# retab-dev/k-LLMs

Hardware: AMD Instinct MI355X
Metric: end_to_end_consensus_requests_per_s (higher is better)
Workload: dtype bf16; 1 GPU; model=llama-3-8b, n=5, mode=create, global_batch=24, seq_len=512, parallelism=dp1 tp1

## Files before the change

### kllms_amd/engine/engine.py

```python

from __future__ import annotations

import os
import time
from dataclasses import dataclass, field
from typing import Any, List, Optional, Tuple

import torch

from ..models.llama import ForwardBatch
from .config import EngineConfig, ModelArchConfig
from .kvcache import PagedKVCache, SequenceKV
from .sampling import SamplingParams
from .shared_prefix import build_shared_prefix_tiles
from .tokenizer import BaseTokenizer, load_tokenizer
from .. import ops


@dataclass
class GenRequest:
    prompt_ids: List[int]
    n: int = 1
    sampling: SamplingParams = field(default_factory=SamplingParams)
    constraint: Optional[Any] = None
# ... 492 lines not shown
            kv_caches=self.kv.layer_caches(),
            **attn,
        )
        hidden = self.model.forward_hidden(torch.tensor(all_ids, dtype=torch.long, device=dev), batch)
        return self.model.compute_logits(hidden[torch.tensor(last_rows, device=dev)])

    def _alloc_with_prefix(self, ids: List[int], prefix_blocks: List[int]) -> SequenceKV:
        if not prefix_blocks:
            return self.kv.alloc_sequence(len(ids))
        bs = self.kv.block_size
        n_total = (len(ids) + bs - 1) // bs
        seq = SequenceKV(blocks=[], num_tokens=len(ids))
        try:
            for b in prefix_blocks:
                self.kv.allocator.incref(b)
                seq.blocks.append(b)
            for _ in range(n_total - len(prefix_blocks)):
                seq.blocks.append(self.kv.allocator.alloc())
        except Exception:
            for b in seq.blocks:
                self.kv.allocator.free(b)
            seq.blocks = []
            raise
        return seq

    def _fork_and_sample(
        self,
        requests: List[GenRequest],
        parent_seqs: List[SequenceKV],
        prefill_logits: torch.Tensor,
        streams: List[_Stream],
    ) -> List[_Stream]:
        new_streams: List[_Stream] = []
        for ri, req in enumerate(requests):
            rid = self._seed_counter
            self._seed_counter += 1
            base_seed = req.sampling.seed if req.sampling.seed is not None else (self.config.seed * 1000003 + rid)
            fork_id = self._fork_counter
            self._fork_counter += 1
            for si in range(max(1, req.n)):
                seq = self.kv.fork(parent_seqs[ri])
                cstate = req.constraint.init_state() if req.constraint is not None else None
                st = _Stream(ri, si, seq, req.sampling, seed=base_seed + 7919 * si,
                             constraint=req.constraint, constraint_state=cstate,
                             fork_id=fork_id)
                st.deadline = req.deadline if self.ctx.world_size == 1 else None
                streams.append(st)
                new_streams.append(st)
            self.kv.free_sequence(parent_seqs[ri])

        rep_logits = torch.cat([
            prefill_logits[ri].unsqueeze(0).expand(max(1, requests[ri].n), -1)
            for ri in range(len(requests))
        ])
        self._sample_and_append(rep_logits.contiguous(), new_streams)
        return new_streams

    def prefill_chunk(
        self, seq: SequenceKV, prompt_ids: List[int], start: int, end: int, want_logits: bool = False
    ) -> Optional[torch.Tensor]:
        dev = self.device
        ids = torch.tensor(prompt_ids[start:end], dtype=torch.long, device=dev)
        pos = torch.arange(start, end, dtype=torch.long, device=dev)
        slots_all = self.kv.prefill_slot_mapping(seq)
        slots = torch.tensor(slots_all[start:end], dtype=torch.long, device=dev)
        if self.paged_prefill_attention:
            attn = dict(extend=ops.build_paged_prefill(
                [end - start], [start], [seq.blocks], dev, self.kv.block_size))
        else:
            nb = len(seq.blocks)
            bt = (
                torch.tensor(seq.blocks, dtype=torch.int32, device=dev)
                .unsqueeze(0).expand(end - start, nb).contiguous()
            )
            attn = dict(block_tables=bt,
                        context_lens=torch.arange(start + 1, end + 1, dtype=torch.int32, device=dev))
        batch = ForwardBatch(
            mode="decode",
            positions=pos,
            slot_mapping=slots,
            kv_caches=self.kv.layer_caches(),
            **attn,
# ... 296 lines not shown
```

### kllms_amd/engine/kvcache.py

```python

from __future__ import annotations

import hashlib
from array import array
from collections import OrderedDict
from dataclasses import dataclass, field
from typing import Callable, List, Optional, Tuple

import torch


class BlockAllocator:
    def __init__(self, num_blocks: int):
        self.num_blocks = num_blocks
        self._free: list[int] = list(range(num_blocks - 1, -1, -1))
        self._refcount = [0] * num_blocks
        self.on_pressure: Optional[Callable[[], None]] = None

    @property
    def num_free(self) -> int:
        return len(self._free)

    def alloc(self) -> int:
        if not self._free and self.on_pressure is not None:
            self.on_pressure()
        if not self._free:
            raise RuntimeError("KV cache out of blocks")
        b = self._free.pop()
        assert self._refcount[b] == 0
        self._refcount[b] = 1
        return b

    def incref(self, block: int) -> None:
        assert self._refcount[block] > 0
        self._refcount[block] += 1

    def free(self, block: int) -> None:
        assert self._refcount[block] > 0
        self._refcount[block] -= 1
        if self._refcount[block] == 0:
            self._free.append(block)

# ... 26 lines not shown
        self.k_all = torch.zeros(num_layers, num_blocks, num_kv_heads, block_size, head_dim,
                                 device=device, dtype=dtype)
        self.v_all = torch.zeros_like(self.k_all)
        self.k_caches = [self.k_all[i] for i in range(num_layers)]
        self.v_caches = [self.v_all[i] for i in range(num_layers)]
        self.fp8 = dtype == torch.float8_e4m3fn
        if self.fp8:
            self.k_scale_all = torch.ones(num_layers, num_blocks, num_kv_heads, block_size,
                                          device=device, dtype=torch.float32)
            self.v_scale_all = torch.ones_like(self.k_scale_all)
        else:
            self.k_scale_all = self.v_scale_all = None
        self.allocator = BlockAllocator(num_blocks)

    def layer_caches(self) -> List[Tuple[torch.Tensor, torch.Tensor, Optional[torch.Tensor], Optional[torch.Tensor]]]:
        if self.fp8:
            return [(self.k_caches[i], self.v_caches[i], self.k_scale_all[i], self.v_scale_all[i])
                    for i in range(self.num_layers)]
        return [(self.k_caches[i], self.v_caches[i], None, None) for i in range(self.num_layers)]

    def alloc_sequence(self, num_tokens: int) -> SequenceKV:
        n_blocks = (num_tokens + self.block_size - 1) // self.block_size
        blocks: List[int] = []
        try:
            for _ in range(n_blocks):
                blocks.append(self.allocator.alloc())
        except Exception:
            for b in blocks:
                self.allocator.free(b)
            raise
        return SequenceKV(blocks=blocks, num_tokens=num_tokens)

    def fork(self, parent: SequenceKV) -> SequenceKV:
        child = SequenceKV(blocks=[], num_tokens=parent.num_tokens)
        tail = parent.num_tokens % self.block_size
        try:
            for i, b in enumerate(parent.blocks):
                if i == len(parent.blocks) - 1 and tail != 0:
                    child.blocks.append(self._copy_block(b))
                else:
                    self.allocator.incref(b)
                    child.blocks.append(b)
        except Exception:
            for b in child.blocks:
                self.allocator.free(b)
            child.blocks = []
            raise
        return child

    def _copy_block(self, src: int) -> int:
        dst = self.allocator.alloc()
        self.k_all[:, dst].copy_(self.k_all[:, src])
        self.v_all[:, dst].copy_(self.v_all[:, src])
        if self.fp8:
            self.k_scale_all[:, dst].copy_(self.k_scale_all[:, src])
            self.v_scale_all[:, dst].copy_(self.v_scale_all[:, src])
        return dst

    def append_slot(self, seq: SequenceKV) -> int:
        pos = seq.num_tokens
        off = pos % self.block_size
        blk_idx = pos // self.block_size
        if blk_idx == len(seq.blocks):
            seq.blocks.append(self.allocator.alloc())
        else:
            last = seq.blocks[blk_idx]
            if self.allocator.refcount(last) > 1:
                new = self._copy_block(last)
                self.allocator.free(last)
                seq.blocks[blk_idx] = new
        seq.num_tokens += 1
        return seq.blocks[blk_idx] * self.block_size + off

    def prefill_slot_mapping(self, seq: SequenceKV, start: int = 0) -> list[int]:
        slots = []
        for pos in range(start, seq.num_tokens):
            slots.append(seq.blocks[pos // self.block_size] * self.block_size + pos % self.block_size)
        return slots

    def free_sequence(self, seq: SequenceKV) -> None:
        for b in seq.blocks:
            self.allocator.free(b)
        seq.blocks = []
        seq.num_tokens = 0


class PrefixCache:

    def __init__(self, kv: "PagedKVCache", max_blocks: int):
# ... 64 lines not shown
```

### kllms_amd/models/llama.py

```python

from __future__ import annotations

import math
from dataclasses import dataclass
from typing import List, Literal, Optional, Tuple

import torch
import torch.nn as nn

from .. import ops
from ..engine.config import ModelArchConfig
from ..ops.torch_ref import build_cos_sin_cache
from ..parallel.tp import ColumnParallelLinear, ParallelContext, RowParallelLinear


@dataclass
class ForwardBatch:
    mode: Literal["prefill", "decode"]
    positions: torch.Tensor
    slot_mapping: torch.Tensor
    kv_caches: List[Tuple]
    cu_seqlens: Optional[torch.Tensor] = None
    block_tables: Optional[torch.Tensor] = None
    context_lens: Optional[torch.Tensor] = None
    shared: Optional["ops.SharedPrefix"] = None
    extend: Optional["ops.PagedPrefill"] = None


class LlamaAttention(nn.Module):
    def __init__(self, cfg: ModelArchConfig, ctx: ParallelContext, layer_idx: int, dtype):
        super().__init__()
        self.layer_idx = layer_idx
        tp = ctx.world_size
        assert cfg.num_heads % tp == 0 and cfg.num_kv_heads % tp == 0
        self.num_heads = cfg.num_heads // tp
        self.num_kv_heads = cfg.num_kv_heads // tp
        self.head_dim = cfg.head_dim_
        self.scale = 1.0 / math.sqrt(self.head_dim)
        q_size = cfg.num_heads * self.head_dim
        kv_size = cfg.num_kv_heads * self.head_dim
        self.qkv_proj = ColumnParallelLinear(
            cfg.hidden_size, q_size + 2 * kv_size, ctx, dtype=dtype,
            partition_sizes=[q_size, kv_size, kv_size],
            bias=cfg.attention_qkv_bias,
        )
        self.o_proj = RowParallelLinear(q_size, cfg.hidden_size, ctx, dtype=dtype)
        self._q = self.num_heads * self.head_dim
        self._kv = self.num_kv_heads * self.head_dim

    def forward(self, hidden: torch.Tensor, batch: ForwardBatch, cos_sin: torch.Tensor) -> torch.Tensor:
        T = hidden.shape[0]
        qkv = self.qkv_proj(hidden)
        q, k, v = qkv.split([self._q, self._kv, self._kv], dim=-1)
        q = q.view(T, self.num_heads, self.head_dim)
        k = k.view(T, self.num_kv_heads, self.head_dim)
        v = v.view(T, self.num_kv_heads, self.head_dim)
        ops.rope_inplace(q, k, batch.positions, cos_sin)

        k_cache, v_cache, k_scale, v_scale = batch.kv_caches[self.layer_idx]
        ops.store_kv(k, v, k_cache, v_cache, batch.slot_mapping, k_scale, v_scale)

        if batch.mode == "prefill":
            out = ops.attn_prefill_varlen(q, k, v, batch.cu_seqlens, self.scale)
        elif batch.extend is not None:
            out = ops.attn_prefill_paged(
                q, k_cache, v_cache, batch.extend, self.scale, k_scale, v_scale)
        else:
            out = ops.attn_decode_paged(
                q, k_cache, v_cache, batch.block_tables, batch.context_lens, self.scale,
                k_scale, v_scale, shared=batch.shared,
            )
        return self.o_proj(out.reshape(T, -1))


class LlamaMLP(nn.Module):
    def __init__(self, cfg: ModelArchConfig, ctx: ParallelContext, dtype):
        super().__init__()
        self.gate_up_proj = ColumnParallelLinear(
            cfg.hidden_size, 2 * cfg.intermediate_size, ctx, dtype=dtype,
            partition_sizes=[cfg.intermediate_size, cfg.intermediate_size],
        )
        self.down_proj = RowParallelLinear(cfg.intermediate_size, cfg.hidden_size, ctx, dtype=dtype)
        self._i = cfg.intermediate_size // ctx.world_size

    def forward(self, x: torch.Tensor) -> torch.Tensor:
        gate_up = self.gate_up_proj(x)
        gate, up = gate_up.split([self._i, self._i], dim=-1)
        return self.down_proj(ops.silu_mul(gate, up))


class RMSNormModule(nn.Module):
    def __init__(self, hidden_size: int, eps: float, dtype):
        super().__init__()
# ... 141 lines not shown
```

### kllms_amd/ops/__init__.py

```python

from __future__ import annotations

import os
from dataclasses import dataclass
from typing import Optional, Tuple

import torch

from . import torch_ref

_C = None
_C_err: Optional[str] = None
try:
    from kllms_amd import _C
except Exception as e:
    _C = None
    _C_err = str(e)


def hip_available() -> bool:
    return _C is not None


def _force_torch() -> bool:
# ... 94 lines not shown
        if x.dtype != torch.bfloat16:
            raise ValueError(f"linear_fp8w_batched on GPU needs bf16 activations, got {x.dtype}")
        if _fp8w_batched_kernel_takes(x, E, N, K):
            out = torch.empty((E, x.shape[-2], N), dtype=torch.bfloat16, device=x.device)
            C.linear_fp8w_batched(out, x, q, scale)
            return out
        if K % 16 == 0:
            w = torch.empty((E, N, K), dtype=torch.bfloat16, device=x.device)
            C.dequant_fp8w(w, q.view(E * N, K), scale.view(E * N))
        else:
            w = (q.float() * scale.unsqueeze(-1)).bfloat16()
        xb = x.unsqueeze(0).expand(E, -1, -1) if x.dim() == 2 else x
        return torch.bmm(xb, w.transpose(1, 2))
    return torch_ref.linear_fp8w_batched(x, q, scale)


def store_kv(
    k: torch.Tensor,
    v: torch.Tensor,
    k_cache: torch.Tensor,
    v_cache: torch.Tensor,
    slot_mapping: torch.Tensor,
    k_scale: Optional[torch.Tensor] = None,
    v_scale: Optional[torch.Tensor] = None,
) -> None:
    if k.is_cuda and not _force_torch():
        none = torch.empty(0, dtype=torch.float32, device=k.device)
        _hip_or_raise().store_kv(
            k, v, k_cache, v_cache, slot_mapping,
            k_scale if k_scale is not None else none,
            v_scale if v_scale is not None else none)
        return
    torch_ref.store_kv(k, v, k_cache, v_cache, slot_mapping, k_scale, v_scale)


def _prefill_tiles(cu_seqlens: torch.Tensor, device) -> tuple:
    NW = 8
    cu = cu_seqlens.cpu().tolist()
    grp_start, grp_len, grp_qpos0 = [], [], []
    for i in range(len(cu) - 1):
        s, e = cu[i], cu[i + 1]
        L = e - s
        tiles = list(range(0, L, 32))
        for g0 in range(0, len(tiles), NW):
            grp_start.append(s)
            grp_len.append(L)
            grp = tiles[g0 : g0 + NW]
            grp_qpos0.extend(grp + [-1] * (NW - len(grp)))
    t = lambda x: torch.tensor(x, dtype=torch.int32, device=device)
    return t(grp_start), t(grp_qpos0), t(grp_len)


def attn_prefill_varlen(
    q: torch.Tensor, k: torch.Tensor, v: torch.Tensor, cu_seqlens: torch.Tensor, scale: float
) -> torch.Tensor:
    if q.is_cuda and not _force_torch():
        out = torch.empty(q.shape, dtype=q.dtype, device=q.device)
        gs, gq, gl = _prefill_tiles(cu_seqlens, q.device)
        _hip_or_raise().attn_prefill(out, q, k, v, gs, gq, gl, scale)
        return out
    return torch_ref.attn_prefill_varlen(q, k, v, cu_seqlens, scale)


@dataclass
class SharedPrefix:

# ... 217 lines not shown
```

### kllms_amd/ops/hip/bindings.hip

```cpp

#include <torch/extension.h>
#include <ATen/hip/HIPContext.h>

#include "common.h"

extern "C" __global__ void rmsnorm_kernel(bf16_t*, const bf16_t*, const bf16_t*, int, float);
extern "C" __global__ void fused_add_rmsnorm_kernel(bf16_t*, const bf16_t*, bf16_t*, const bf16_t*, int, float);
extern "C" __global__ void silu_mul_kernel(bf16_t*, const bf16_t*, const bf16_t*, int64_t, int, int);
extern "C" __global__ void rope_kernel(bf16_t*, bf16_t*, const int64_t*, const float*, int, int, int, int, int);
extern "C" __global__ void store_kv_kernel(const bf16_t*, const bf16_t*, bf16_t*, bf16_t*, const int64_t*, int, int, int, int, int);
extern "C" __global__ void store_kv_fp8_kernel(const bf16_t*, const bf16_t*, unsigned char*, unsigned char*, float*, float*, const int64_t*, int, int, int, int, int);
extern "C" void launch_attn_decode_partial(float*, const bf16_t*, const void*, const void*, const float*, const float*, const int*, const int*, const int*, float, int, int, int, int, int, int, int, int, int, hipStream_t);
extern "C" void launch_attn_decode_shared(float*, const bf16_t*, const void*, const void*, const float*, const float*, const int*, const int*, const int*, const int*, float, int, int, int, int, int, int, int, int, int, int, hipStream_t);
extern "C" void launch_attn_prefill_paged(bf16_t*, const bf16_t*, const void*, const void*, const float*, const float*, const int*, const int*, const int*, const int*, const int*, float, int, int, int, int, int, int, int, int, int, int, hipStream_t);
extern "C" __global__ void attn_decode_reduce_kernel(bf16_t*, const float*, const int*, int, int, int, int);
extern "C" __global__ void attn_prefill_kernel(bf16_t*, const bf16_t*, const bf16_t*, const bf16_t*, const int*, const int*, const int*, float, int, int, int, int);
extern "C" __global__ void sample_kernel(int64_t*, float*, const float*, const float*, const float*, const int*, const int64_t*, const int64_t*, const uint32_t*, int, float*);
extern "C" __global__ void sample_fsm_kernel(int64_t*, float*, const float*, const float*, const float*, const int*, const int64_t*, const int64_t*, int32_t*, const int64_t*, int, int);
extern "C" __global__ void mfma_selftest_kernel(float*, const bf16_t*, const bf16_t*);

#define CHECK_BF16_CONTIG(t) \
  TORCH_CHECK((t).is_cuda() && (t).is_contiguous() && (t).scalar_type() == at::kBFloat16, #t " must be contiguous bf16 on GPU")

#define CHECK_KV_CACHE(t) \
  TORCH_CHECK((t).is_cuda() && (t).is_contiguous() && \
              ((t).scalar_type() == at::kBFloat16 || (t).scalar_type() == at::kFloat8_e4m3fn), \
              #t " must be a contiguous bf16 or fp8-e4m3 KV cache on GPU")

#define CHECK_BF16_ROWS(t) \
  TORCH_CHECK((t).is_cuda() && (t).scalar_type() == at::kBFloat16 && (t).dim() == 3 && \
              (t).stride(2) == 1 && (t).stride(1) == (t).size(2), #t " must be a bf16 [T,H,D] row view")

static inline hipStream_t cur_stream() {
  return at::hip::getCurrentHIPStream().stream();
}

static bf16_t* bf(torch::Tensor& t) { return reinterpret_cast<bf16_t*>(t.data_ptr()); }
static const bf16_t* cbf(const torch::Tensor& t) { return reinterpret_cast<const bf16_t*>(t.data_ptr()); }

void rmsnorm(torch::Tensor out, torch::Tensor in, torch::Tensor weight, double eps) {
  CHECK_BF16_CONTIG(out); CHECK_BF16_CONTIG(in); CHECK_BF16_CONTIG(weight);
  const int n = in.size(-1);
  TORCH_CHECK(n % 8 == 0, "hidden size must be a multiple of 8");
  const int rows = in.numel() / n;
// ... 28 lines not shown
  CHECK_BF16_ROWS(q); CHECK_BF16_ROWS(k);
  TORCH_CHECK(positions.scalar_type() == at::kLong && cos_sin.scalar_type() == at::kFloat);
  const int T = q.size(0), H = q.size(1), D = q.size(2), KVH = k.size(1);
  hipLaunchKernelGGL(rope_kernel, dim3(T, H + KVH), dim3(D / 2), 0, cur_stream(),
                     bf(q), bf(k), positions.data_ptr<int64_t>(), cos_sin.data_ptr<float>(),
                     H, KVH, D, (int)q.stride(0), (int)k.stride(0));
}

void store_kv(torch::Tensor k, torch::Tensor v, torch::Tensor k_cache, torch::Tensor v_cache,
              torch::Tensor slot_mapping, torch::Tensor k_scale, torch::Tensor v_scale) {
  CHECK_BF16_ROWS(k); CHECK_BF16_ROWS(v); CHECK_KV_CACHE(k_cache); CHECK_KV_CACHE(v_cache);
  TORCH_CHECK(k.stride(0) == v.stride(0), "k/v must share the token stride");
  const int T = k.size(0), KVH = k.size(1), D = k.size(2);
  const int BS = k_cache.size(2);
  if (k_cache.scalar_type() == at::kFloat8_e4m3fn) {
    TORCH_CHECK(k_scale.numel() == k_cache.size(0) * KVH * BS && k_scale.is_contiguous() &&
                    k_scale.scalar_type() == at::kFloat && v_scale.numel() == k_scale.numel(),
                "fp8 store_kv requires [NB, KVH, BS] fp32 k_scale/v_scale");
    const int64_t rows = (int64_t)T * KVH;
    const int grid = (int)std::min<int64_t>((rows + 3) / 4, 2048);
    hipLaunchKernelGGL(store_kv_fp8_kernel, dim3(grid), dim3(256), 0, cur_stream(),
                       cbf(k), cbf(v),
                       reinterpret_cast<unsigned char*>(k_cache.data_ptr()),
                       reinterpret_cast<unsigned char*>(v_cache.data_ptr()),
                       k_scale.data_ptr<float>(), v_scale.data_ptr<float>(),
                       slot_mapping.data_ptr<int64_t>(), T, KVH, D, BS, (int)k.stride(0));
  } else {
    const int64_t total = (int64_t)T * KVH * (D / 8);
    const int grid = (int)std::min<int64_t>((total + 255) / 256, 2048);
    hipLaunchKernelGGL(store_kv_kernel, dim3(grid), dim3(256), 0, cur_stream(),
                       cbf(k), cbf(v), bf(k_cache), bf(v_cache),
                       slot_mapping.data_ptr<int64_t>(), T, KVH, D, BS, (int)k.stride(0));
  }
}

static void attn_decode_paged_impl(torch::Tensor& out, torch::Tensor& q, torch::Tensor& k_cache,
                                   torch::Tensor& v_cache, torch::Tensor& block_tables,
                                   torch::Tensor& context_lens, double scale,
                                   torch::Tensor& k_scale, torch::Tensor& v_scale, bool shared,
                                   const int* skip_chunks, const int* tile_rows,
                                   const int* tile_nmembers, const int* tile_chunks,
                                   int n_tiles) {
  CHECK_BF16_CONTIG(out); CHECK_BF16_ROWS(q); CHECK_KV_CACHE(k_cache); CHECK_KV_CACHE(v_cache);
  const int B = q.size(0), H = q.size(1), D = q.size(2);
  const int KVH = k_cache.size(1), BS = k_cache.size(2);
  TORCH_CHECK(D == 128, "attn_decode: head_dim must be 128");
  TORCH_CHECK(H % KVH == 0, "attn_decode: H must be a multiple of KVH");
  TORCH_CHECK(H / KVH == 1 || H / KVH == 2 || H / KVH == 4 || H / KVH == 8,
              "attn_decode: GQA group must be 1, 2, 4 or 8");
  const int gqa = H / KVH;
  const int max_blocks = block_tables.size(1);
  const int max_ctx = max_blocks * BS;
  const int CHUNK_KEYS = ATTN_DECODE_TKV;
  const int max_chunks = std::max(1, (max_ctx + CHUNK_KEYS - 1) / CHUNK_KEYS);
  auto partials = torch::empty({(int64_t)B * KVH * max_chunks * gqa * 130},
                               torch::dtype(torch::kFloat).device(q.device()));
  const int cache_fp8 = k_cache.scalar_type() == at::kFloat8_e4m3fn ? 1 : 0;
  if (cache_fp8) {
    TORCH_CHECK(k_scale.numel() == k_cache.size(0) * KVH * BS && k_scale.is_contiguous() &&
                    k_scale.scalar_type() == at::kFloat && v_scale.numel() == k_scale.numel(),
                "fp8 attn_decode requires [NB, KVH, BS] fp32 k_scale/v_scale");
  }
  if (shared && n_tiles > 0) {
    launch_attn_decode_shared(
        partials.data_ptr<float>(), cbf(q), k_cache.data_ptr(), v_cache.data_ptr(),
        cache_fp8 ? k_scale.data_ptr<float>() : nullptr,
// ... 394 lines not shown
                             scale.data_ptr<float>(), (int)E, (int)M, (int)N, (int)K,
                             (long)x_stride, (long)x_bstride, mt, splitk, cur_stream());
}

void dequant_fp8w(torch::Tensor w, torch::Tensor q, torch::Tensor scale) {
  CHECK_FP8W(q, scale);
  CHECK_BF16_CONTIG(w);
  TORCH_CHECK(w.numel() >= q.numel(), "dequant_fp8w: scratch smaller than the weight");
  TORCH_CHECK(q.size(1) % 16 == 0, "dequant_fp8w: K must be a multiple of 16");
  TORCH_CHECK(reinterpret_cast<uintptr_t>(q.data_ptr()) % 16 == 0 &&
              reinterpret_cast<uintptr_t>(w.data_ptr()) % 16 == 0,
              "dequant_fp8w: q and w must be 16-byte aligned");
  if (q.numel() == 0) return;
  launch_dequant_fp8w(w.data_ptr(), q.data_ptr(), scale.data_ptr<float>(), (long)q.numel(),
                      (int)q.size(1), cur_stream());
}

PYBIND11_MODULE(TORCH_EXTENSION_NAME, m) {
  m.def("linear_fp8w", &linear_fp8w);
  m.def("linear_fp8w_batched", &linear_fp8w_batched);
  m.def("dequant_fp8w", &dequant_fp8w);
  m.def("levenshtein_pairs", &levenshtein_pairs);
  m.def("moe_gateup", &moe_gateup);
  m.def("moe_down", &moe_down);
  m.def("ipc_allreduce_create", &ipc_allreduce_create);
  m.def("ipc_allreduce_connect", &ipc_allreduce_connect);
  m.def("ipc_allreduce_run", &ipc_allreduce_run);
  m.def("ipc_allreduce_destroy", &ipc_allreduce_destroy);
  m.def("rmsnorm", &rmsnorm);
  m.def("fused_add_rmsnorm", &fused_add_rmsnorm);
  m.def("silu_mul", &silu_mul);
  m.def("rope_inplace", &rope_inplace);
  m.def("store_kv", &store_kv);
  m.def("attn_decode_paged", &attn_decode_paged);
  m.def("attn_decode_paged_shared", &attn_decode_paged_shared);
  m.def("attn_prefill", &attn_prefill);
  m.def("attn_prefill_paged", &attn_prefill_paged);
  m.def("sample", &sample);
  m.def("sample_fsm", &sample_fsm);
  m.def("mfma_selftest", &mfma_selftest);
  m.def("one_shot_allreduce", &one_shot_allreduce);
}
```

### kllms_amd/ops/hip/elementwise.hip

```cpp

#include "common.h"

extern "C" __global__ void __launch_bounds__(256) rmsnorm_kernel(
    bf16_t* __restrict__ out, const bf16_t* __restrict__ in,
    const bf16_t* __restrict__ w, int n, float eps) {
  __shared__ float red[16];
  const int row = blockIdx.x;
  const bf16x8_vec* inv = reinterpret_cast<const bf16x8_vec*>(in + (int64_t)row * n);
  bf16x8_vec* outv = reinterpret_cast<bf16x8_vec*>(out + (int64_t)row * n);
  const bf16x8_vec* wv = reinterpret_cast<const bf16x8_vec*>(w);
  const int nvec = n / 8;

  float ss = 0.0f;
  for (int i = threadIdx.x; i < nvec; i += blockDim.x) {
    bf16x8_vec v = inv[i];
#pragma unroll
    for (int j = 0; j < 8; ++j) {
      float f = bf16_to_f32(v[j]);
      ss += f * f;
    }
  }
  ss = block_reduce_sum<4>(ss, red);
  const float inv_rms = rsqrtf(ss / n + eps);

  for (int i = threadIdx.x; i < nvec; i += blockDim.x) {
    bf16x8_vec v = inv[i];
    bf16x8_vec wv8 = wv[i];
    bf16x8_vec o;
#pragma unroll
    for (int j = 0; j < 8; ++j)
      o[j] = f32_to_bf16(bf16_to_f32(v[j]) * inv_rms * bf16_to_f32(wv8[j]));
    outv[i] = o;
  }
}

extern "C" __global__ void __launch_bounds__(256) fused_add_rmsnorm_kernel(
    bf16_t* __restrict__ out, const bf16_t* __restrict__ x,
    bf16_t* __restrict__ residual, const bf16_t* __restrict__ w, int n, float eps) {
  __shared__ float red[16];
  const int row = blockIdx.x;
  const bf16x8_vec* xv = reinterpret_cast<const bf16x8_vec*>(x + (int64_t)row * n);
  bf16x8_vec* rv = reinterpret_cast<bf16x8_vec*>(residual + (int64_t)row * n);
  bf16x8_vec* outv = reinterpret_cast<bf16x8_vec*>(out + (int64_t)row * n);
  const bf16x8_vec* wv = reinterpret_cast<const bf16x8_vec*>(w);
  const int nvec = n / 8;

  float ss = 0.0f;
  for (int i = threadIdx.x; i < nvec; i += blockDim.x) {
    bf16x8_vec a = xv[i];
    bf16x8_vec b = rv[i];
    bf16x8_vec s;
#pragma unroll
    for (int j = 0; j < 8; ++j) {
      float f = bf16_to_f32(a[j]) + bf16_to_f32(b[j]);
      s[j] = f32_to_bf16(f);
      float fs = bf16_to_f32(s[j]);
      ss += fs * fs;
    }
    rv[i] = s;
  }
  ss = block_reduce_sum<4>(ss, red);
  const float inv_rms = rsqrtf(ss / n + eps);

  for (int i = threadIdx.x; i < nvec; i += blockDim.x) {
    bf16x8_vec s = rv[i];
    bf16x8_vec wv8 = wv[i];
    bf16x8_vec o;
#pragma unroll
    for (int j = 0; j < 8; ++j)
      o[j] = f32_to_bf16(bf16_to_f32(s[j]) * inv_rms * bf16_to_f32(wv8[j]));
    outv[i] = o;
  }
}

extern "C" __global__ void __launch_bounds__(256) silu_mul_kernel(
    bf16_t* __restrict__ out, const bf16_t* __restrict__ gate,
    const bf16_t* __restrict__ up, int64_t nvec, int ncols_vec, int row_stride_vec) {
  bf16x8_vec* ov = reinterpret_cast<bf16x8_vec*>(out);
  for (int64_t i = blockIdx.x * blockDim.x + threadIdx.x; i < nvec;
       i += (int64_t)gridDim.x * blockDim.x) {
    const int64_t row = i / ncols_vec;
    const int64_t col = i % ncols_vec;
    const int64_t src = row * row_stride_vec + col;
    bf16x8_vec g = reinterpret_cast<const bf16x8_vec*>(gate)[src];
    bf16x8_vec u = reinterpret_cast<const bf16x8_vec*>(up)[src];
    bf16x8_vec o;
#pragma unroll
    for (int j = 0; j < 8; ++j) {
      float gf = bf16_to_f32(g[j]);
      float s = gf / (1.0f + __expf(-gf));
      o[j] = f32_to_bf16(s * bf16_to_f32(u[j]));
    }
// ... 55 lines not shown
    unsigned char* __restrict__ k_cache, unsigned char* __restrict__ v_cache,
    float* __restrict__ k_scale, float* __restrict__ v_scale,
    const int64_t* __restrict__ slots, int num_tokens, int kv_heads,
    int head_dim, int block_size, int kv_tstride) {
  const int64_t rows = (int64_t)num_tokens * kv_heads;
  const int lane = threadIdx.x & 63;
  for (int64_t row = blockIdx.x * 4 + (threadIdx.x >> 6); row < rows;
       row += (int64_t)gridDim.x * 4) {
    const int g = row % kv_heads;
    const int t = row / kv_heads;
    const int64_t slot = slots[t];
    const int64_t blk = slot / block_size;
    const int off = slot % block_size;
    const bf16_t* src_k = k + (int64_t)t * kv_tstride + g * head_dim;
    const bf16_t* src_v = v + (int64_t)t * kv_tstride + g * head_dim;
    float amax_k = 0.f, amax_v = 0.f;
    for (int d = lane; d < head_dim; d += 64) {
      amax_k = fmaxf(amax_k, fabsf(bf16_to_f32(((const short*)src_k)[d])));
      amax_v = fmaxf(amax_v, fabsf(bf16_to_f32(((const short*)src_v)[d])));
    }
    const float sk = fmaxf(wave_reduce_max(amax_k) * (1.0f / 448.0f), 1e-8f);
    const float sv = fmaxf(wave_reduce_max(amax_v) * (1.0f / 448.0f), 1e-8f);
    const int64_t srow = (blk * kv_heads + g) * block_size + off;
    if (lane == 0) { k_scale[srow] = sk; v_scale[srow] = sv; }
    const float isk = 1.0f / sk, isv = 1.0f / sv;
    unsigned char* dst_k = k_cache + srow * head_dim;
    unsigned char* dst_v = v_cache + srow * head_dim;
    for (int d = lane; d < head_dim; d += 64) {
      dst_k[d] = f32_to_fp8(bf16_to_f32(((const short*)src_k)[d]) * isk);
      dst_v[d] = f32_to_fp8(bf16_to_f32(((const short*)src_v)[d]) * isv);
    }
  }
}
```

### setup.py

```python

import os

from setuptools import setup

os.environ.setdefault("PYTORCH_ROCM_ARCH", "gfx950")

from torch.utils.cpp_extension import BuildExtension, CUDAExtension

HIP_DIR = os.path.join("kllms_amd", "ops", "hip")
SOURCES = [
    os.path.join(HIP_DIR, f)
    for f in (
        "bindings.hip",
        "elementwise.hip",
        "attn_decode.hip",
        "attn_decode_shared.hip",
        "attn_prefill.hip",
        "attn_prefill_paged.hip",
        "sampling.hip",
        "mfma_selftest.hip",
        "allreduce.hip",
        "moe.hip",
        "levenshtein.hip",
        "linear_fp8w.hip",
    )
]

setup(
    name="kllms_amd_C",
    ext_modules=[
        CUDAExtension(
            name="kllms_amd._C",
            sources=SOURCES,
            extra_compile_args={
                "cxx": ["-O3"],
                "nvcc": ["-O3", "--offload-arch=gfx950", "-std=c++17"],
            },
        )
    ],
    cmdclass={"build_ext": BuildExtension},
)
```

Before: 31.98 req/s.

## Batch KV fork copies, fuse RoPE with KV store, register-cache add-rmsnorm

Replaces the per-child tail-block copy during fork with a single batched copy kernel over all (src,dst) pairs, instead of several strided torch copies per child. Fuses RoPE and the KV cache store into one kernel, so each layer issues one launch and writes rotated K straight into the cache. Adds a register-resident fast path to fused add-rmsnorm that avoids rereading the residual. The changes add host-side assertions and a host-to-device tensor transfer for the copy pairs, and change the rounding order inside rmsnorm.

```diff
diff --git a/kllms_amd/engine/engine.py b/kllms_amd/engine/engine.py
--- a/kllms_amd/engine/engine.py
+++ b/kllms_amd/engine/engine.py
@@ -548,6 +548,8 @@
         streams: List[_Stream],
     ) -> List[_Stream]:
         new_streams: List[_Stream] = []
+        forked = self.kv.fork_batch(
+            [(parent_seqs[ri], max(1, req.n)) for ri, req in enumerate(requests)])
         for ri, req in enumerate(requests):
             rid = self._seed_counter
             self._seed_counter += 1
@@ -555,15 +557,23 @@
             fork_id = self._fork_counter
             self._fork_counter += 1
             for si in range(max(1, req.n)):
-                seq = self.kv.fork(parent_seqs[ri])
-                cstate = req.constraint.init_state() if req.constraint is not None else None
-                st = _Stream(ri, si, seq, req.sampling, seed=base_seed + 7919 * si,
-                             constraint=req.constraint, constraint_state=cstate,
-                             fork_id=fork_id)
+                seq = forked[ri][si]
+                try:
+                    cstate = req.constraint.init_state() if req.constraint is not None else None
+                    st = _Stream(ri, si, seq, req.sampling, seed=base_seed + 7919 * si,
+                                 constraint=req.constraint, constraint_state=cstate,
+                                 fork_id=fork_id)
+                except Exception:
+                    for children in forked:
+                        for child in children:
+                            if child.blocks and all(child is not s.seq for s in new_streams):
+                                self.kv.free_sequence(child)
+                    raise
                 st.deadline = req.deadline if self.ctx.world_size == 1 else None
                 streams.append(st)
                 new_streams.append(st)
-            self.kv.free_sequence(parent_seqs[ri])
+        for seq in parent_seqs[:len(requests)]:
+            self.kv.free_sequence(seq)
 
         rep_logits = torch.cat([
             prefill_logits[ri].unsqueeze(0).expand(max(1, requests[ri].n), -1)
diff --git a/kllms_amd/engine/kvcache.py b/kllms_amd/engine/kvcache.py
--- a/kllms_amd/engine/kvcache.py
+++ b/kllms_amd/engine/kvcache.py
@@ -8,6 +8,8 @@
 from typing import Callable, List, Optional, Tuple
 
 import torch
+
+from .. import ops
 
 
 class BlockAllocator:
@@ -100,29 +102,55 @@
         return SequenceKV(blocks=blocks, num_tokens=num_tokens)
 
     def fork(self, parent: SequenceKV) -> SequenceKV:
-        child = SequenceKV(blocks=[], num_tokens=parent.num_tokens)
-        tail = parent.num_tokens % self.block_size
+        return self.fork_batch([(parent, 1)])[0][0]
+
+    def fork_batch(self, parents_and_counts) -> List[List[SequenceKV]]:
+        out: List[List[SequenceKV]] = []
+        src: List[int] = []
+        dst: List[int] = []
         try:
-            for i, b in enumerate(parent.blocks):
-                if i == len(parent.blocks) - 1 and tail != 0:
-                    child.blocks.append(self._copy_block(b))
-                else:
-                    self.allocator.incref(b)
-                    child.blocks.append(b)
+            for parent, count in parents_and_counts:
+                tail = parent.num_tokens % self.block_size
+                last = len(parent.blocks) - 1
+                children: List[SequenceKV] = []
+                out.append(children)
+                for _ in range(count):
+                    child = SequenceKV(blocks=[], num_tokens=parent.num_tokens)
+                    children.append(child)
+                    for i, b in enumerate(parent.blocks):
+                        if i == last and tail != 0:
+                            child.blocks.append(self.allocator.alloc())
+                            src.append(b)
+                            dst.append(child.blocks[-1])
+                        else:
+                            self.allocator.incref(b)
+                            child.blocks.append(b)
         except Exception:
-            for b in child.blocks:
-                self.allocator.free(b)
-            child.blocks = []
+            for children in out:
+                for child in children:
+                    for b in child.blocks:
+                        self.allocator.free(b)
+                    child.blocks = []
             raise
-        return child
+        self._copy_blocks(src, dst)
+        return out
+
+    def _copy_blocks(self, src: List[int], dst: List[int]) -> None:
+        if not src:
+            return
+        assert len(src) == len(dst)
+        assert all(0 <= b < self.num_blocks for b in src) and \
+            all(0 <= b < self.num_blocks for b in dst), "block id out of range"
+        assert len(set(dst)) == len(dst), "a block is the destination of two copies"
+        assert set(src).isdisjoint(dst), "a block is both a source and a destination"
+        pairs = torch.tensor([src, dst], dtype=torch.int32).to(self.k_all.device)
+        ops.copy_kv_blocks(self.k_all, self.v_all, pairs[0], pairs[1])
+        if self.fp8:
+            ops.copy_kv_blocks(self.k_scale_all, self.v_scale_all, pairs[0], pairs[1])
 
     def _copy_block(self, src: int) -> int:
         dst = self.allocator.alloc()
-        self.k_all[:, dst].copy_(self.k_all[:, src])
-        self.v_all[:, dst].copy_(self.v_all[:, src])
-        if self.fp8:
-            self.k_scale_all[:, dst].copy_(self.k_scale_all[:, src])
-            self.v_scale_all[:, dst].copy_(self.v_scale_all[:, src])
+        self._copy_blocks([src], [dst])
         return dst
 
     def append_slot(self, seq: SequenceKV) -> int:
diff --git a/kllms_amd/models/llama.py b/kllms_amd/models/llama.py
--- a/kllms_amd/models/llama.py
+++ b/kllms_amd/models/llama.py
@@ -55,10 +55,9 @@
         q = q.view(T, self.num_heads, self.head_dim)
         k = k.view(T, self.num_kv_heads, self.head_dim)
         v = v.view(T, self.num_kv_heads, self.head_dim)
-        ops.rope_inplace(q, k, batch.positions, cos_sin)
-
         k_cache, v_cache, k_scale, v_scale = batch.kv_caches[self.layer_idx]
-        ops.store_kv(k, v, k_cache, v_cache, batch.slot_mapping, k_scale, v_scale)
+        ops.rope_store_kv(q, k, v, batch.positions, cos_sin, k_cache, v_cache,
+                          batch.slot_mapping, k_scale, v_scale)
 
         if batch.mode == "prefill":
             out = ops.attn_prefill_varlen(q, k, v, batch.cu_seqlens, self.scale)
diff --git a/kllms_amd/ops/__init__.py b/kllms_amd/ops/__init__.py
--- a/kllms_amd/ops/__init__.py
+++ b/kllms_amd/ops/__init__.py
@@ -150,6 +150,41 @@
             v_scale if v_scale is not None else none)
         return
     torch_ref.store_kv(k, v, k_cache, v_cache, slot_mapping, k_scale, v_scale)
+
+
+def rope_store_kv(
+    q: torch.Tensor,
+    k: torch.Tensor,
+    v: torch.Tensor,
+    positions: torch.Tensor,
+    cos_sin: torch.Tensor,
+    k_cache: torch.Tensor,
+    v_cache: torch.Tensor,
+    slot_mapping: torch.Tensor,
+    k_scale: Optional[torch.Tensor] = None,
+    v_scale: Optional[torch.Tensor] = None,
+) -> None:
+    if q.is_cuda and not _force_torch():
+        none = torch.empty(0, dtype=torch.float32, device=q.device)
+        _hip_or_raise().rope_store_kv(
+            q, k, v, positions, cos_sin, k_cache, v_cache, slot_mapping,
+            k_scale if k_scale is not None else none,
+            v_scale if v_scale is not None else none)
+        return
+    torch_ref.rope_inplace(q, k, positions, cos_sin)
+    torch_ref.store_kv(k, v, k_cache, v_cache, slot_mapping, k_scale, v_scale)
+
+
+def copy_kv_blocks(a_all: torch.Tensor, b_all: torch.Tensor,
+                   src: torch.Tensor, dst: torch.Tensor) -> None:
+    if src.numel() == 0:
+        return
+    if a_all.is_cuda and not _force_torch():
+        _hip_or_raise().copy_kv_blocks(a_all, b_all, src, dst)
+        return
+    s, d = src.long(), dst.long()
+    a_all[:, d] = a_all[:, s]
+    b_all[:, d] = b_all[:, s]
 
 
 def _prefill_tiles(cu_seqlens: torch.Tensor, device) -> tuple:
diff --git a/kllms_amd/ops/hip/bindings.hip b/kllms_amd/ops/hip/bindings.hip
--- a/kllms_amd/ops/hip/bindings.hip
+++ b/kllms_amd/ops/hip/bindings.hip
@@ -10,6 +10,9 @@
 extern "C" __global__ void rope_kernel(bf16_t*, bf16_t*, const int64_t*, const float*, int, int, int, int, int);
 extern "C" __global__ void store_kv_kernel(const bf16_t*, const bf16_t*, bf16_t*, bf16_t*, const int64_t*, int, int, int, int, int);
 extern "C" __global__ void store_kv_fp8_kernel(const bf16_t*, const bf16_t*, unsigned char*, unsigned char*, float*, float*, const int64_t*, int, int, int, int, int);
+extern "C" __global__ void rope_store_kv_kernel(bf16_t*, bf16_t*, const bf16_t*, bf16_t*, bf16_t*, const int64_t*, const float*, const int64_t*, int, int, int, int, int, int, int);
+extern "C" __global__ void rope_store_kv_fp8_kernel(bf16_t*, bf16_t*, const bf16_t*, unsigned char*, unsigned char*, float*, float*, const int64_t*, const float*, const int64_t*, int, int, int, int, int, int, int);
+extern "C" void launch_copy_kv_blocks(void*, void*, const int*, const int*, int, int, int64_t, int64_t, int, hipStream_t);
 extern "C" void launch_attn_decode_partial(float*, const bf16_t*, const void*, const void*, const float*, const float*, const int*, const int*, const int*, float, int, int, int, int, int, int, int, int, int, hipStream_t);
 extern "C" void launch_attn_decode_shared(float*, const bf16_t*, const void*, const void*, const float*, const float*, const int*, const int*, const int*, const int*, float, int, int, int, int, int, int, int, int, int, int, hipStream_t);
 extern "C" void launch_attn_prefill_paged(bf16_t*, const bf16_t*, const void*, const void*, const float*, const float*, const int*, const int*, const int*, const int*, const int*, float, int, int, int, int, int, int, int, int, int, int, hipStream_t);
@@ -104,6 +107,77 @@
                        cbf(k), cbf(v), bf(k_cache), bf(v_cache),
                        slot_mapping.data_ptr<int64_t>(), T, KVH, D, BS, (int)k.stride(0));
   }
+}
+
+void rope_store_kv(torch::Tensor q, torch::Tensor k, torch::Tensor v, torch::Tensor positions,
+                   torch::Tensor cos_sin, torch::Tensor k_cache, torch::Tensor v_cache,
+                   torch::Tensor slot_mapping, torch::Tensor k_scale, torch::Tensor v_scale) {
+  CHECK_BF16_ROWS(q); CHECK_BF16_ROWS(k); CHECK_BF16_ROWS(v);
+  CHECK_KV_CACHE(k_cache); CHECK_KV_CACHE(v_cache);
+  TORCH_CHECK(positions.is_cuda() && positions.scalar_type() == at::kLong && positions.is_contiguous() &&
+              cos_sin.is_cuda() && cos_sin.scalar_type() == at::kFloat && cos_sin.is_contiguous(),
+              "rope_store_kv: positions must be int64 and cos_sin fp32, contiguous on GPU");
+  TORCH_CHECK(slot_mapping.is_cuda() && slot_mapping.scalar_type() == at::kLong &&
+              slot_mapping.is_contiguous(), "rope_store_kv: slot_mapping must be contiguous int64 on GPU");
+  const int T = q.size(0), H = q.size(1), D = q.size(2), KVH = k.size(1);
+  TORCH_CHECK(k.size(0) == T && v.size(0) == T && k.size(2) == D && v.size(2) == D &&
+              v.size(1) == KVH, "rope_store_kv: q/k/v disagree on T, KVH or D");
+  TORCH_CHECK(positions.numel() == T && slot_mapping.numel() == T,
+              "rope_store_kv: positions and slot_mapping must be [T]");
+  TORCH_CHECK(k_cache.dim() == 4 && v_cache.sizes() == k_cache.sizes() &&
+              v_cache.scalar_type() == k_cache.scalar_type() && k_cache.size(1) == KVH &&
+              k_cache.size(3) == D && cos_sin.size(-1) == D,
+              "rope_store_kv: caches must be [NB, KVH, BS, D] of one dtype, cos_sin [max_pos, D]");
+  TORCH_CHECK(D % 8 == 0 && v.stride(0) % 8 == 0 &&
+              reinterpret_cast<uintptr_t>(v.data_ptr()) % 16 == 0,
+              "rope_store_kv: head_dim must be a multiple of 8 and v rows 16-byte aligned");
+  if (T == 0) return;
+  const int BS = k_cache.size(2);
+  const dim3 grid(T, (H + KVH + 3) / 4);
+  if (k_cache.scalar_type() == at::kFloat8_e4m3fn) {
+    TORCH_CHECK(k_scale.is_cuda() && v_scale.is_cuda() &&
+                    k_scale.numel() == k_cache.size(0) * KVH * BS && k_scale.is_contiguous() &&
+                    v_scale.is_contiguous() && k_scale.scalar_type() == at::kFloat &&
+                    v_scale.scalar_type() == at::kFloat && v_scale.numel() == k_scale.numel(),
+                "fp8 rope_store_kv requires [NB, KVH, BS] fp32 k_scale/v_scale");
+    hipLaunchKernelGGL(rope_store_kv_fp8_kernel, grid, dim3(256), 0, cur_stream(),
+                       bf(q), bf(k), cbf(v),
+                       reinterpret_cast<unsigned char*>(k_cache.data_ptr()),
+                       reinterpret_cast<unsigned char*>(v_cache.data_ptr()),
+                       k_scale.data_ptr<float>(), v_scale.data_ptr<float>(),
+                       positions.data_ptr<int64_t>(), cos_sin.data_ptr<float>(),
+                       slot_mapping.data_ptr<int64_t>(), H, KVH, D, BS,
+                       (int)q.stride(0), (int)k.stride(0), (int)v.stride(0));
+  } else {
+    hipLaunchKernelGGL(rope_store_kv_kernel, grid, dim3(256), 0, cur_stream(),
+                       bf(q), bf(k), cbf(v), bf(k_cache), bf(v_cache),
+                       positions.data_ptr<int64_t>(), cos_sin.data_ptr<float>(),
+                       slot_mapping.data_ptr<int64_t>(), H, KVH, D, BS,
+                       (int)q.stride(0), (int)k.stride(0), (int)v.stride(0));
+  }
+}
+
+void copy_kv_blocks(torch::Tensor a, torch::Tensor b, torch::Tensor src, torch::Tensor dst) {
+  TORCH_CHECK(a.is_cuda() && b.is_cuda() && a.is_contiguous() && b.is_contiguous() &&
+              a.dim() >= 2 && a.sizes() == b.sizes() && a.scalar_type() == b.scalar_type(),
+              "copy_kv_blocks: a/b must be contiguous [L, NB, ...] GPU arrays of one shape and dtype");
+  auto ok = [&](const torch::Tensor& t) {
+    return t.is_cuda() && t.device() == a.device() && t.is_contiguous() &&
+           t.scalar_type() == at::kInt && t.dim() == 1;
+  };
+  TORCH_CHECK(ok(src) && ok(dst) && src.numel() == dst.numel(),
+              "copy_kv_blocks: src/dst must be contiguous int32 [n] on the arrays' device");
+  const int64_t n = src.numel(), L = a.size(0), NB = a.size(1);
+  if (n == 0 || L == 0 || NB == 0) return;
+  TORCH_CHECK(n <= INT32_MAX / 2 / L, "copy_kv_blocks: too many pairs");
+  const int64_t block_bytes = a.stride(1) * (int64_t)a.element_size();
+  const int64_t layer_stride = a.stride(0) * (int64_t)a.element_size();
+  const uintptr_t bits = reinterpret_cast<uintptr_t>(a.data_ptr()) |
+                         reinterpret_cast<uintptr_t>(b.data_ptr()) |
+                         (uintptr_t)block_bytes | (uintptr_t)layer_stride;
+  const int vec = bits % 16 == 0 ? 16 : (bits % 4 == 0 ? 4 : 1);
+  launch_copy_kv_blocks(a.data_ptr(), b.data_ptr(), src.data_ptr<int>(), dst.data_ptr<int>(),
+                        (int)n, (int)L, layer_stride, block_bytes, vec, cur_stream());
 }
 
 static void attn_decode_paged_impl(torch::Tensor& out, torch::Tensor& q, torch::Tensor& k_cache,
@@ -564,6 +638,8 @@
   m.def("silu_mul", &silu_mul);
   m.def("rope_inplace", &rope_inplace);
   m.def("store_kv", &store_kv);
+  m.def("rope_store_kv", &rope_store_kv);
+  m.def("copy_kv_blocks", &copy_kv_blocks);
   m.def("attn_decode_paged", &attn_decode_paged);
   m.def("attn_decode_paged_shared", &attn_decode_paged_shared);
   m.def("attn_prefill", &attn_prefill);
diff --git a/kllms_amd/ops/hip/elementwise.hip b/kllms_amd/ops/hip/elementwise.hip
--- a/kllms_amd/ops/hip/elementwise.hip
+++ b/kllms_amd/ops/hip/elementwise.hip
@@ -33,6 +33,33 @@
     outv[i] = o;
   }
 }
+
+__device__ __forceinline__ float add_square(float ss, float f) {
+#pragma clang fp contract(off)
+  const float sq = f * f;
+  return ss + sq;
+}
+
+__device__ __forceinline__ bf16x8_vec add_round_vec(bf16x8_vec a, bf16x8_vec b, float& ss) {
+  bf16x8_vec s;
+#pragma unroll
+  for (int j = 0; j < 8; ++j) {
+    float f = bf16_to_f32(a[j]) + bf16_to_f32(b[j]);
+    s[j] = f32_to_bf16(f);
+    ss = add_square(ss, bf16_to_f32(s[j]));
+  }
+  return s;
+}
+
+__device__ __forceinline__ bf16x8_vec scale_vec(bf16x8_vec s, bf16x8_vec w8, float inv_rms) {
+  bf16x8_vec o;
+#pragma unroll
+  for (int j = 0; j < 8; ++j)
+    o[j] = f32_to_bf16(bf16_to_f32(s[j]) * inv_rms * bf16_to_f32(w8[j]));
+  return o;
+}
+
+#define ADD_RMSNORM_REG_VECS 4
 
 extern "C" __global__ void __launch_bounds__(256) fused_add_rmsnorm_kernel(
     bf16_t* __restrict__ out, const bf16_t* __restrict__ x,
@@ -46,18 +73,33 @@
   const int nvec = n / 8;
 
   float ss = 0.0f;
+  if (nvec <= ADD_RMSNORM_REG_VECS * (int)blockDim.x) {
+    bf16x8_vec s[ADD_RMSNORM_REG_VECS], wr[ADD_RMSNORM_REG_VECS];
+#pragma unroll
+    for (int u = 0; u < ADD_RMSNORM_REG_VECS; ++u) {
+      const int i = threadIdx.x + u * blockDim.x;
+      if (i < nvec) {
+        bf16x8_vec a = xv[i];
+        bf16x8_vec b = rv[i];
+        wr[u] = wv[i];
+        s[u] = add_round_vec(a, b, ss);
+        rv[i] = s[u];
+      }
+    }
+    ss = block_reduce_sum<4>(ss, red);
+    const float inv_rms = rsqrtf(ss / n + eps);
+#pragma unroll
+    for (int u = 0; u < ADD_RMSNORM_REG_VECS; ++u) {
+      const int i = threadIdx.x + u * blockDim.x;
+      if (i < nvec) outv[i] = scale_vec(s[u], wr[u], inv_rms);
+    }
+    return;
+  }
+
   for (int i = threadIdx.x; i < nvec; i += blockDim.x) {
     bf16x8_vec a = xv[i];
     bf16x8_vec b = rv[i];
-    bf16x8_vec s;
-#pragma unroll
-    for (int j = 0; j < 8; ++j) {
-      float f = bf16_to_f32(a[j]) + bf16_to_f32(b[j]);
-      s[j] = f32_to_bf16(f);
-      float fs = bf16_to_f32(s[j]);
-      ss += fs * fs;
-    }
-    rv[i] = s;
+    rv[i] = add_round_vec(a, b, ss);
   }
   ss = block_reduce_sum<4>(ss, red);
   const float inv_rms = rsqrtf(ss / n + eps);
@@ -179,3 +221,135 @@
     }
   }
 }
+
+
+__device__ __forceinline__ float rope_first(float x1, float x2, float c, float s) {
+#pragma clang fp contract(off)
+  const float p = x2 * s;
+  return __builtin_fmaf(x1, c, -p);
+}
+
+__device__ __forceinline__ float rope_second(float x1, float x2, float c, float s) {
+#pragma clang fp contract(off)
+  const float p = x2 * c;
+  return __builtin_fmaf(x1, s, p);
+}
+
+template <bool FP8>
+__device__ __forceinline__ void rope_store_kv_body(
+    bf16_t* __restrict__ q, bf16_t* __restrict__ k, const bf16_t* __restrict__ v,
+    void* __restrict__ k_cache, void* __restrict__ v_cache,
+    float* __restrict__ k_scale, float* __restrict__ v_scale,
+    const int64_t* __restrict__ positions, const float* __restrict__ cos_sin,
+    const int64_t* __restrict__ slots, int num_q_heads, int num_kv_heads, int head_dim,
+    int block_size, int q_tstride, int k_tstride, int v_tstride) {
+  const int t = blockIdx.x;
+  const int h = blockIdx.y * 4 + (threadIdx.x >> 6);
+  const int lane = threadIdx.x & 63;
+  if (h >= num_q_heads + num_kv_heads) return;
+  const int half = head_dim / 2;
+  const int64_t pos = positions[t];
+  const float* cs = cos_sin + pos * head_dim;
+  const bool is_k = h >= num_q_heads;
+  const int g = h - num_q_heads;
+  short* base = reinterpret_cast<short*>(
+      is_k ? k + (int64_t)t * k_tstride + g * head_dim : q + (int64_t)t * q_tstride + h * head_dim);
+
+  if (!is_k) {
+    for (int i = lane; i < half; i += 64) {
+      const float c = cs[i], s = cs[half + i];
+      const float x1 = bf16_to_f32(base[i]), x2 = bf16_to_f32(base[half + i]);
+      base[i] = f32_to_bf16(rope_first(x1, x2, c, s));
+      base[half + i] = f32_to_bf16(rope_second(x1, x2, c, s));
+    }
+    return;
+  }
+
+  const int64_t slot = slots[t];
+  const int64_t blk = slot / block_size;
+  const int off = slot % block_size;
+  const int64_t srow = (blk * num_kv_heads + g) * block_size + off;
+  const short* src_v = reinterpret_cast<const short*>(v + (int64_t)t * v_tstride + g * head_dim);
+
+  if (!FP8) {
+    short* dst_k = reinterpret_cast<short*>(k_cache) + srow * head_dim;
+    for (int i = lane; i < half; i += 64) {
+      const float c = cs[i], s = cs[half + i];
+      const float x1 = bf16_to_f32(base[i]), x2 = bf16_to_f32(base[half + i]);
+      const short r1 = f32_to_bf16(rope_first(x1, x2, c, s));
+      const short r2 = f32_to_bf16(rope_second(x1, x2, c, s));
+      base[i] = r1;
+      base[half + i] = r2;
+      dst_k[i] = r1;
+      dst_k[half + i] = r2;
+    }
+    bf16x8_vec* dst_v = reinterpret_cast<bf16x8_vec*>(reinterpret_cast<short*>(v_cache) + srow * head_dim);
+    for (int dv = lane; dv < head_dim / 8; dv += 64)
+      dst_v[dv] = reinterpret_cast<const bf16x8_vec*>(src_v)[dv];
+    return;
+  }
+
+  float amax_k = 0.f, amax_v = 0.f;
+  auto rotate = [&](int i, short& r1, short& r2) {
+    const float c = cs[i], s = cs[half + i];
+    const float x1 = bf16_to_f32(base[i]), x2 = bf16_to_f32(base[half + i]);
+    r1 = f32_to_bf16(rope_first(x1, x2, c, s));
+    r2 = f32_to_bf16(rope_second(x1, x2, c, s));
+    base[i] = r1;
+    base[half + i] = r2;
+    amax_k = fmaxf(amax_k, fabsf(bf16_to_f32(r1)));
+    amax_k = fmaxf(amax_k, fabsf(bf16_to_f32(r2)));
+  };
+  short ra1 = 0, ra2 = 0, rb1 = 0, rb2 = 0;
+  if (lane < half) rotate(lane, ra1, ra2);
+  if (lane + 64 < half) rotate(lane + 64, rb1, rb2);
+  for (int i = lane + 128; i < half; i += 64) {
+    short r1, r2;
+    rotate(i, r1, r2);
+  }
+  for (int d = lane; d < head_dim; d += 64)
+    amax_v = fmaxf(amax_v, fabsf(bf16_to_f32(src_v[d])));
+  const float sk = fmaxf(wave_reduce_max(amax_k) * (1.0f / 448.0f), 1e-8f);
+  const float sv = fmaxf(wave_reduce_max(amax_v) * (1.0f / 448.0f), 1e-8f);
+  if (lane == 0) { k_scale[srow] = sk; v_scale[srow] = sv; }
+  const float isk = 1.0f / sk, isv = 1.0f / sv;
+  unsigned char* dst_k = reinterpret_cast<unsigned char*>(k_cache) + srow * head_dim;
+  unsigned char* dst_v = reinterpret_cast<unsigned char*>(v_cache) + srow * head_dim;
+  if (lane < half) {
+    dst_k[lane] = f32_to_fp8(bf16_to_f32(ra1) * isk);
+    dst_k[half + lane] = f32_to_fp8(bf16_to_f32(ra2) * isk);
+  }
+  if (lane + 64 < half) {
+    dst_k[lane + 64] = f32_to_fp8(bf16_to_f32(rb1) * isk);
+    dst_k[half + lane + 64] = f32_to_fp8(bf16_to_f32(rb2) * isk);
+  }
+  for (int i = lane + 128; i < half; i += 64) {
+    dst_k[i] = f32_to_fp8(bf16_to_f32(base[i]) * isk);
+    dst_k[half + i] = f32_to_fp8(bf16_to_f32(base[half + i]) * isk);
+  }
+  for (int d = lane; d < head_dim; d += 64)
+    dst_v[d] = f32_to_fp8(bf16_to_f32(src_v[d]) * isv);
+}
+
+extern "C" __global__ void __launch_bounds__(256) rope_store_kv_kernel(
+    bf16_t* __restrict__ q, bf16_t* __restrict__ k, const bf16_t* __restrict__ v,
+    bf16_t* __restrict__ k_cache, bf16_t* __restrict__ v_cache,
+    const int64_t* __restrict__ positions, const float* __restrict__ cos_sin,
+    const int64_t* __restrict__ slots, int num_q_heads, int num_kv_heads, int head_dim,
+    int block_size, int q_tstride, int k_tstride, int v_tstride) {
+  rope_store_kv_body<false>(q, k, v, k_cache, v_cache, nullptr, nullptr, positions, cos_sin,
+                            slots, num_q_heads, num_kv_heads, head_dim, block_size,
+                            q_tstride, k_tstride, v_tstride);
+}
+
+extern "C" __global__ void __launch_bounds__(256) rope_store_kv_fp8_kernel(
+    bf16_t* __restrict__ q, bf16_t* __restrict__ k, const bf16_t* __restrict__ v,
+    unsigned char* __restrict__ k_cache, unsigned char* __restrict__ v_cache,
+    float* __restrict__ k_scale, float* __restrict__ v_scale,
+    const int64_t* __restrict__ positions, const float* __restrict__ cos_sin,
+    const int64_t* __restrict__ slots, int num_q_heads, int num_kv_heads, int head_dim,
+    int block_size, int q_tstride, int k_tstride, int v_tstride) {
+  rope_store_kv_body<true>(q, k, v, k_cache, v_cache, k_scale, v_scale, positions, cos_sin,
+                           slots, num_q_heads, num_kv_heads, head_dim, block_size,
+                           q_tstride, k_tstride, v_tstride);
+}
diff --git a/kllms_amd/ops/hip/kv_copy.hip b/kllms_amd/ops/hip/kv_copy.hip
--- /dev/null
+++ b/kllms_amd/ops/hip/kv_copy.hip
@@ -0,0 +1,52 @@
+
+#include "common.h"
+
+#define KV_COPY_MAX_GRID 2048
+
+template <typename VEC>
+__global__ void __launch_bounds__(256) copy_kv_blocks_kernel(
+    unsigned char* __restrict__ a_base, unsigned char* __restrict__ b_base,
+    const int* __restrict__ src, const int* __restrict__ dst, int n_pairs, int n_layers,
+    int64_t layer_stride, int64_t block_bytes) {
+  const int64_t units = (int64_t)n_pairs * n_layers * 2;
+  const int64_t nvec = block_bytes / (int64_t)sizeof(VEC);
+  for (int64_t u = blockIdx.x; u < units; u += gridDim.x) {
+    const int which = (int)(u & 1);
+    const int64_t pl = u >> 1;
+    const int layer = (int)(pl % n_layers);
+    const int pair = (int)(pl / n_layers);
+    unsigned char* base = (which ? b_base : a_base) + (int64_t)layer * layer_stride;
+    const VEC* s = reinterpret_cast<const VEC*>(base + (int64_t)src[pair] * block_bytes);
+    VEC* d = reinterpret_cast<VEC*>(base + (int64_t)dst[pair] * block_bytes);
+    const int64_t bd = blockDim.x;
+    int64_t i = threadIdx.x;
+    for (; i + 3 * bd < nvec; i += 4 * bd) {
+      const VEC v0 = s[i], v1 = s[i + bd], v2 = s[i + 2 * bd], v3 = s[i + 3 * bd];
+      d[i] = v0;
+      d[i + bd] = v1;
+      d[i + 2 * bd] = v2;
+      d[i + 3 * bd] = v3;
+    }
+    for (; i < nvec; i += bd) d[i] = s[i];
+  }
+}
+
+extern "C" void launch_copy_kv_blocks(void* a_base, void* b_base, const int* src, const int* dst,
+                                      int n_pairs, int n_layers, int64_t layer_stride,
+                                      int64_t block_bytes, int vec_bytes, hipStream_t stream) {
+  const int64_t units = (int64_t)n_pairs * n_layers * 2;
+  if (units <= 0 || block_bytes <= 0) return;
+  const int grid = (int)(units < KV_COPY_MAX_GRID ? units : KV_COPY_MAX_GRID);
+  unsigned char* a = reinterpret_cast<unsigned char*>(a_base);
+  unsigned char* b = reinterpret_cast<unsigned char*>(b_base);
+  if (vec_bytes == 16) {
+    hipLaunchKernelGGL(copy_kv_blocks_kernel<fw_u32x4>, dim3(grid), dim3(256), 0, stream,
+                       a, b, src, dst, n_pairs, n_layers, layer_stride, block_bytes);
+  } else if (vec_bytes == 4) {
+    hipLaunchKernelGGL(copy_kv_blocks_kernel<unsigned int>, dim3(grid), dim3(256), 0, stream,
+                       a, b, src, dst, n_pairs, n_layers, layer_stride, block_bytes);
+  } else {
+    hipLaunchKernelGGL(copy_kv_blocks_kernel<unsigned char>, dim3(grid), dim3(256), 0, stream,
+                       a, b, src, dst, n_pairs, n_layers, layer_stride, block_bytes);
+  }
+}
diff --git a/setup.py b/setup.py
--- a/setup.py
+++ b/setup.py
@@ -13,6 +13,7 @@
     for f in (
         "bindings.hip",
         "elementwise.hip",
+        "kv_copy.hip",
         "attn_decode.hip",
         "attn_decode_shared.hip",
         "attn_prefill.hip",
```

After: 33.28 req/s, median of 6. 4.1% higher.
